# pierotofy/OpenSplat

Hardware: NVIDIA H100
Metric: fwd_bwd_mpixel_per_s (higher is better)
Workload: dtype f32

## Files before the change

### opensplat_b200/csrc/raster_bwd.cu

```cuda
#include "raster_common.cuh"

int gsb_blend_grid(const void *kernel, int num_tiles);

namespace {

__device__ __forceinline__ float rcp_approx(float x) {
    float y;
    asm("rcp.approx.ftz.f32 %0, %1;" : "=f"(y) : "f"(x));
    return y;
}

__device__ __forceinline__ void zero_row(float *grad_rows, int k) {
    float4 *row = reinterpret_cast<float4 *>(grad_rows + (size_t)k * GSB_GRAD_ROW_FLOATS);
    const float4 z = make_float4(0.f, 0.f, 0.f, 0.f);
    row[0] = z; row[1] = z; row[2] = z;
}

constexpr int BWD_MIN_BLOCKS = 6;
constexpr int BWD_DEPTH_MIN_BLOCKS = 5;
constexpr int BWD_ABS_MIN_BLOCKS = 5;
constexpr int BWD_DEPTH_ABS_MIN_BLOCKS = 4;
template <bool SAT, bool DEPTH, bool ABS>
__global__ void __launch_bounds__(RK_THREADS, ABS ? (DEPTH ? BWD_DEPTH_ABS_MIN_BLOCKS : BWD_ABS_MIN_BLOCKS)
                                                  : (DEPTH ? BWD_DEPTH_MIN_BLOCKS : BWD_MIN_BLOCKS))
rasterize_backward_kernel(int img_h, int img_w, int tiles_x, int num_tiles,
                          const int2 *__restrict__ tile_bins, const GsbRecord *__restrict__ records,
                          const float *__restrict__ background, const float *__restrict__ final_Ts,
                          const int *__restrict__ final_idx, const float *__restrict__ v_output,
                          const float *__restrict__ v_output_alpha, float *__restrict__ grad_rows,
                          unsigned *__restrict__ tile_counter, const int *__restrict__ tile_order,
                          const float *__restrict__ record_depths, const float *__restrict__ v_output_depth) {
    __shared__ WarpRing rings[RK_WARPS];
    const int warp = threadIdx.x >> 5, lane = threadIdx.x & 31;
    WarpRing &ring = rings[warp];
    if (lane == 0) {
#pragma unroll
        for (int s = 0; s < RK_STAGES; ++s) mbar_init(&ring.full[s], 1);
        mbar_fence_init();
    }
    __syncwarp();
    const float bg0 = __ldg(background), bg1 = __ldg(background + 1), bg2 = __ldg(background + 2);
    unsigned gchunk = 0;

    while (true) {
        int tile = 0;
        if (lane == 0) tile = (int)atomicAdd(tile_counter, 1u);
        tile = __shfl_sync(0xffffffffu, tile, 0);
        if (tile >= num_tiles) break;
        if (tile_order) tile = __ldg(tile_order + tile);
        const int2 range = tile_bins[tile];
        if (range.y <= range.x) continue;

        const int tx = tile % tiles_x, ty = tile / tiles_x;
        const int X = tx * GSB_TILE + (lane & 15);
        const int Y0 = ty * GSB_TILE + (lane >> 4);
        const float px = (float)X;
        const float tile_x0 = (float)(tx * GSB_TILE), tile_y0 = (float)(ty * GSB_TILE);

        float T[RK_PIX], Bq[RK_PIX];
        const float py0 = (float)Y0;
        float vor[RK_PIX], vog[RK_PIX], vob[RK_PIX];
        float vD[RK_PIX];
        int binf[RK_PIX];
        int my_max = -1;
#pragma unroll
        for (int j = 0; j < RK_PIX; ++j) {
            const int Y = Y0 + 2 * j;
            if (X < img_w && Y < img_h) {
                const size_t p = (size_t)Y * img_w + X;
                const float Tf = final_Ts[p];
                T[j] = Tf;
                vor[j] = v_output[3 * p]; vog[j] = v_output[3 * p + 1]; vob[j] = v_output[3 * p + 2];
                binf[j] = final_idx[p];
                if (SAT) {
                    const int f = binf[j];
                    if (f & GSB_SAT_BIT0) vor[j] = 0.f;
                    if (f & (GSB_SAT_BIT0 << 1)) vog[j] = 0.f;
                    if (f & (GSB_SAT_BIT0 << 2)) vob[j] = 0.f;
                    binf[j] = f & ~GSB_SAT_MASK;
                }
                if (DEPTH) vD[j] = v_output_depth ? v_output_depth[p] : 0.f;
                const float voa = v_output_alpha ? v_output_alpha[p] : 0.f;
                Bq[j] = -(Tf * (voa - (bg0 * vor[j] + bg1 * vog[j] + bg2 * vob[j])));
            } else {
                T[j] = 1.f; vor[j] = vog[j] = vob[j] = 0.f; Bq[j] = 0.f;
                if (DEPTH) vD[j] = 0.f;
                binf[j] = -1;
            }
            my_max = max(my_max, binf[j]);
        }
        const int warp_max = __reduce_max_sync(0xffffffffu, my_max);
        const int hi = min(range.y - 1, max(warp_max, range.x - 1));

        for (int idx = hi + 1 + lane; idx < range.y; idx += 32)
            zero_row(grad_rows, __float_as_int(__ldg(&records[idx].q0.w)));
        const int L = hi - range.x + 1;
        if (L <= 0) continue;
        const int nchunks = (L + RK_CHUNK - 1) / RK_CHUNK;

        const unsigned g0 = gchunk;
        auto stage_of = [&](int c) { return (g0 + (unsigned)c) % RK_STAGES; };
        auto parity_of = [&](int c) { return ((g0 + (unsigned)c) / RK_STAGES) & 1u; };
        auto chunk_lo = [&](int c) { return max(range.x, hi + 1 - (c + 1) * RK_CHUNK); };
        auto chunk_cnt = [&](int c) { return (hi + 1 - c * RK_CHUNK) - chunk_lo(c); };
        auto issue = [&](int c) {
            if (lane == 0) {
                const unsigned s = stage_of(c);
                const uint32_t bytes = (uint32_t)chunk_cnt(c) * (uint32_t)sizeof(GsbRecord);
                mbar_arrive_expect_tx(&ring.full[s], bytes);
                tma_load_1d(&ring.rec[s][0], records + chunk_lo(c), bytes, &ring.full[s]);
            }
        };
        const int pro = min(RK_STAGES, nchunks);
        for (int c = 0; c < pro; ++c) issue(c);
        int issued = pro;

        for (int c = 0; c < nchunks; ++c) {
            const unsigned s = stage_of(c);
            float zl = 0.f;
            if (DEPTH && lane < chunk_cnt(c)) zl = __ldg(record_depths + chunk_lo(c) + lane);
            mbar_wait(&ring.full[s], parity_of(c));
            const int lo = chunk_lo(c), cnt = chunk_cnt(c);
            unsigned my_mask = 0;
            if (lane < cnt) {
                my_mask = record_slot_mask(ring.rec[s][lane], tile_x0, tile_y0);
                if (my_mask == 0u) zero_row(grad_rows, __float_as_int(ring.rec[s][lane].q0.w));
            }
            unsigned live = __ballot_sync(0xffffffffu, my_mask != 0u);
            while (live) {
                const int t = 31 - __clz(live);
                live &= ~(1u << t);
                const unsigned rm = __shfl_sync(0xffffffffu, my_mask, t);
                float z = 0.f;
                if (DEPTH) z = __shfl_sync(0xffffffffu, zl, t);
                const int idx = lo + t;
                const float4 q0 = ring.rec[s][t].q0;
                const float4 q1 = ring.rec[s][t].q1;
                const float4 q2 = ring.rec[s][t].q2;
                const float smax = fmaxf(0.f, fmaf(q0.z, GSB_LN2, GSB_SMAX_BIAS));
                const float dx = q0.x - px;
                const float adx2 = q1.x * dx * dx;
                const float bdx = q1.y * dx;
                const float dy0 = q0.y - py0;
                float s0 = 0.f, s1 = 0.f, s2 = 0.f;
                float a_r = 0.f, a_g = 0.f, a_b = 0.f;
                float a_z = 0.f;
                float g_x = 0.f, g_y = 0.f;
                float adx = 0.f, c2 = 0.f;
                if (ABS) { adx = (2.f * q1.x) * dx; c2 = 2.f * q1.z; }
                bool any = false;
                const int jlo = __ffs(rm) - 1, jhi = 31 - __clz(rm);
#define GSB_BWD_SLOT(j)                                                                                   \
    {                                                                                                     \
        const float dy = dy0 - (float)(2 * j);                                                                      \
        const float sigma = fmaf(dy, fmaf(q1.z, dy, bdx), adx2);                                          \
        if (__float_as_uint(sigma) <= __float_as_uint(smax)) {                    \
            const float au = ex2_approx(fmaf(sigma, -GSB_LOG2E, q0.z));           \
            const float alpha = fminf(0.99f, au);                                                         \
            if (idx <= binf[j] && alpha >= (1.f / 255.f)) {                                               \
                any = true;                                                                               \
                const float ra = rcp_approx(1.f - alpha);                                                 \
                T[j] *= ra;                                                                               \
                const float fac = alpha * T[j];                                                           \
                a_r = fmaf(fac, vor[j], a_r);                                                             \
                a_g = fmaf(fac, vog[j], a_g);                                                             \
                a_b = fmaf(fac, vob[j], a_b);                                                             \
                if (DEPTH) a_z = fmaf(fac, vD[j], a_z);                                                   \
                float d = fmaf(q2.z, vob[j], fmaf(q2.y, vog[j], q2.x * vor[j]));         \
                if (DEPTH) d = fmaf(z, vD[j], d);                                        \
                const float v_alpha = fmaf(d, T[j], -(ra * Bq[j]));                                       \
                Bq[j] = fmaf(d, fac, Bq[j]);                                                              \
                 \
                const float w = au * v_alpha;                                                             \
                const float wdy = w * dy;                                                                 \
                s0 += w;                                                                                  \
                s1 += wdy;                                                                                \
                s2 = fmaf(wdy, dy, s2);                                                                   \
                if (ABS) {                                                                                \
                    g_x = fmaf(fabsf(w), fabsf(fmaf(q1.y, dy, adx)), g_x);                                \
                    g_y = fmaf(fabsf(w), fabsf(fmaf(c2, dy, bdx)), g_y);                                  \
                }                                                                                         \
            }                                                                                             \
        }                                                                                                 \
        if (jhi == j) break;                                                                              \
    }
                switch (jlo) {
                    case 0: GSB_BWD_SLOT(0)
                    case 1: GSB_BWD_SLOT(1)
                    case 2: GSB_BWD_SLOT(2)
                    case 3: GSB_BWD_SLOT(3)
                    case 4: GSB_BWD_SLOT(4)
                    case 5: GSB_BWD_SLOT(5)
                    case 6: GSB_BWD_SLOT(6)
                    default: GSB_BWD_SLOT(7)
                }
#undef GSB_BWD_SLOT
                const int k = __float_as_int(q0.w);
                float *row = grad_rows + (size_t)k * GSB_GRAD_ROW_FLOATS;
                if (!__any_sync(0xffffffffu, any)) {
                    if (lane < (ABS ? 12 : DEPTH ? 10 : 9)) row[lane] = 0.f;
                    continue;
                }
                const float sx = dx * s0;
                float v0 = s0, v1 = sx, v2 = s1, v3 = dx * sx, v4 = dx * s1, v5 = s2, v6 = a_r, v7 = a_g;
                float v8 = a_b;
                {
                    const bool up = lane & 16;
                    const float t0 = up ? v0 : v4, t1 = up ? v1 : v5, t2 = up ? v2 : v6, t3 = up ? v3 : v7;
                    const float k0 = up ? v4 : v0, k1 = up ? v5 : v1, k2 = up ? v6 : v2, k3 = up ? v7 : v3;
                    v0 = k0 + __shfl_xor_sync(0xffffffffu, t0, 16);
                    v1 = k1 + __shfl_xor_sync(0xffffffffu, t1, 16);
                    v2 = k2 + __shfl_xor_sync(0xffffffffu, t2, 16);
                    v3 = k3 + __shfl_xor_sync(0xffffffffu, t3, 16);
                }
                {
                    const bool up = lane & 8;
                    const float t0 = up ? v0 : v2, t1 = up ? v1 : v3;
                    const float k0 = up ? v2 : v0, k1 = up ? v3 : v1;
                    v0 = k0 + __shfl_xor_sync(0xffffffffu, t0, 8);
                    v1 = k1 + __shfl_xor_sync(0xffffffffu, t1, 8);
                }
                {
                    const bool up = lane & 4;
                    const float t0 = up ? v0 : v1;
                    const float k0 = up ? v1 : v0;
                    v0 = k0 + __shfl_xor_sync(0xffffffffu, t0, 4);
                }
                v0 += __shfl_xor_sync(0xffffffffu, v0, 2);
                v0 += __shfl_xor_sync(0xffffffffu, v0, 1);
                if (ABS) {
                    const bool up = lane & 16;
                    const float t8 = up ? v8 : a_z, k8 = up ? a_z : v8;
                    const float tg = up ? g_x : g_y, kg = up ? g_y : g_x;
                    v8 = k8 + __shfl_xor_sync(0xffffffffu, t8, 16);
                    const float e = kg + __shfl_xor_sync(0xffffffffu, tg, 16);
                    const bool up8 = lane & 8;
                    const float t = up8 ? v8 : e, kk = up8 ? e : v8;
                    v8 = kk + __shfl_xor_sync(0xffffffffu, t, 8);
#pragma unroll
                    for (int o = 4; o > 0; o >>= 1) v8 += __shfl_xor_sync(0xffffffffu, v8, o);
                    const bool wx = (lane & 7) == 1 && (DEPTH || lane != 17);
                    if (((lane & 3) == 0) || wx) row[wx ? 8 + ((lane >> 3) & 1) * 2 + (lane >> 4) : (lane >> 2)] =
                        wx ? v8 : v0;
                } else if (DEPTH) {
                    const bool up = lane & 16;
                    const float t8 = up ? v8 : a_z, k8 = up ? a_z : v8;
                    v8 = k8 + __shfl_xor_sync(0xffffffffu, t8, 16);
#pragma unroll
                    for (int o = 8; o > 0; o >>= 1) v8 += __shfl_xor_sync(0xffffffffu, v8, o);
                    const bool w8 = (lane == 1), w9 = (lane == 17);
                    if (((lane & 3) == 0) || w8 || w9) row[w8 ? 8 : w9 ? 9 : (lane >> 2)] = (w8 || w9) ? v8 : v0;
                } else {
#pragma unroll
                    for (int o = 16; o > 0; o >>= 1) v8 += __shfl_xor_sync(0xffffffffu, v8, o);
                    const bool w8 = (lane == 1);
                    if (((lane & 3) == 0) || w8) row[w8 ? 8 : (lane >> 2)] = w8 ? v8 : v0;
                }
            }
            __syncwarp();
            if (issued < nchunks) { issue(issued); ++issued; }
        }
        gchunk = g0 + (unsigned)issued;
        __syncwarp();
    }
}

template <bool DEPTH, bool ABS>
__global__ void __launch_bounds__(256)
reduce_grad_rows_kernel(int n, const int *__restrict__ cum_tiles_hit, const float *__restrict__ grad_rows,
                        const float *__restrict__ conics, const float *__restrict__ opacities,
                        float2 *__restrict__ v_xy, float *__restrict__ v_conic,
                        float *__restrict__ v_colors, float *__restrict__ v_opacity, float *__restrict__ v_depths,
                        float2 *__restrict__ v_xy_abs) {
    const int g = blockIdx.x * blockDim.x + threadIdx.x;
    if (g >= n) return;
    const int k0 = g ? cum_tiles_hit[g - 1] : 0, k1 = cum_tiles_hit[g];
    float a[9] = {0.f, 0.f, 0.f, 0.f, 0.f, 0.f, 0.f, 0.f, 0.f};
    float az = 0.f;
    float ax = 0.f, ay = 0.f;
    for (int k = k0; k < k1; ++k) {
        const float4 *row = reinterpret_cast<const float4 *>(grad_rows + (size_t)k * GSB_GRAD_ROW_FLOATS);
        const float4 r0 = row[0], r1 = row[1];
        a[0] += r0.x; a[1] += r0.y; a[2] += r0.z; a[3] += r0.w;
        a[4] += r1.x; a[5] += r1.y; a[6] += r1.z; a[7] += r1.w;
        if (ABS) {
            const float4 r2 = row[2];
            a[8] += r2.x;
            if (DEPTH) az += r2.y;
            ax += r2.z; ay += r2.w;
        } else {
            a[8] += reinterpret_cast<const float *>(row)[8];
            if (DEPTH) az += reinterpret_cast<const float *>(row)[9];
        }
    }
    const float S0 = a[0], Sx = a[1], Sy = a[2], Sxx = a[3], Sxy = a[4], Syy = a[5];
    const float ca = conics[3 * g], cb = conics[3 * g + 1], cc = conics[3 * g + 2];
    const float op = opacities[g];
    v_xy[g] = make_float2(-(ca * Sx + cb * Sy), -(cb * Sx + cc * Sy));
    v_conic[3 * g] = -0.5f * Sxx; v_conic[3 * g + 1] = -0.5f * Sxy; v_conic[3 * g + 2] = -0.5f * Syy;
    v_colors[3 * g] = a[6]; v_colors[3 * g + 1] = a[7]; v_colors[3 * g + 2] = a[8];
    v_opacity[g] = (op > 0.f) ? S0 / op : 0.f;
    if (DEPTH) v_depths[g] = az;
    if (ABS) v_xy_abs[g] = make_float2(ax, ay);
}

}

extern "C" size_t gsb_raster_grad_rows_bytes(int m) {
    return gsb_align_up((size_t)(m > 0 ? m : 0) * GSB_GRAD_ROW_FLOATS * 4 + 256, 256);
}

static int backward(int img_h, int img_w, int tiles_x, int tiles_y, int n, int m, const int32_t *tile_bins,
                    const int32_t *tile_order, const float *conics, const float *opacities, void *records,
                    const int32_t *cum_tiles_hit, const float *background, const float *final_Ts,
                    const int32_t *final_idx, const float *v_output, const float *v_output_alpha, void *grad_rows,
                    float *v_xy, float *v_conic, float *v_colors, float *v_opacity, unsigned flags, bool depth,
                    const float *record_depths, const float *v_output_depth, float *v_depths, float *v_xy_abs,
                    gsb_stream_t stream) {
    GSB_CHECK_ARG(img_h > 0 && img_w > 0 && n >= 0 && m >= 0);
    GSB_CHECK_ARG((flags & ~(unsigned)GSB_RASTER_CLAMP_MAX_ONE) == 0);
    const bool sat = (flags & GSB_RASTER_CLAMP_MAX_ONE) != 0;
    GSB_CHECK_ARG(tiles_x == gsb_div_up(img_w, GSB_TILE) && tiles_y == gsb_div_up(img_h, GSB_TILE));
    if (n == 0) return 0;
    GSB_CHECK_ARG(tile_bins && conics && opacities && cum_tiles_hit && background && final_Ts && final_idx &&
                  v_output && v_xy && v_conic && v_colors && v_opacity);
    GSB_CHECK_ARG(!depth || (v_depths && (record_depths || m == 0)));
    GSB_CHECK_ARG(((uintptr_t)v_xy % 8) == 0 && ((uintptr_t)v_xy_abs % 8) == 0);
    const bool abs = v_xy_abs != nullptr;
    cudaStream_t s = (cudaStream_t)stream;
    if (m > 0) {
        GSB_CHECK_ARG(records && grad_rows && ((uintptr_t)records % 16) == 0 && ((uintptr_t)grad_rows % 16) == 0);
        unsigned *counters = reinterpret_cast<unsigned *>(
            reinterpret_cast<char *>(records) + gsb_raster_records_bytes(m) - 256);
        GSB_CUDA(cudaMemsetAsync(counters, 0, 256, s));
        const int num_tiles = tiles_x * tiles_y;
#define GSB_BWD_LAUNCH(S, D, A)                                                                                 \
    rasterize_backward_kernel<S, D, A><<<gsb_blend_grid((const void *)rasterize_backward_kernel<S, D, A>,       \
                                                        num_tiles), RK_THREADS, 0, s>>>(                        \
        img_h, img_w, tiles_x, num_tiles, reinterpret_cast<const int2 *>(tile_bins),                            \
        reinterpret_cast<const GsbRecord *>(records), background, final_Ts, final_idx, v_output, v_output_alpha, \
        reinterpret_cast<float *>(grad_rows), counters, tile_order, record_depths, v_output_depth)
        if (abs) {
            if (depth) {
                if (sat) GSB_BWD_LAUNCH(true, true, true); else GSB_BWD_LAUNCH(false, true, true);
            } else {
                if (sat) GSB_BWD_LAUNCH(true, false, true); else GSB_BWD_LAUNCH(false, false, true);
            }
        } else if (depth) {
            if (sat) GSB_BWD_LAUNCH(true, true, false); else GSB_BWD_LAUNCH(false, true, false);
        } else {
            if (sat) GSB_BWD_LAUNCH(true, false, false); else GSB_BWD_LAUNCH(false, false, false);
        }
#undef GSB_BWD_LAUNCH
    }
#define GSB_REDUCE_LAUNCH(D, A)                                                                                 \
    reduce_grad_rows_kernel<D, A><<<gsb_div_up(n, 256), 256, 0, s>>>(                                           \
        n, cum_tiles_hit, reinterpret_cast<const float *>(grad_rows), conics, opacities,                        \
        reinterpret_cast<float2 *>(v_xy), v_conic, v_colors, v_opacity, v_depths,                               \
        reinterpret_cast<float2 *>(v_xy_abs))
    if (abs) {
        if (depth) GSB_REDUCE_LAUNCH(true, true); else GSB_REDUCE_LAUNCH(false, true);
    } else if (depth) {
        GSB_REDUCE_LAUNCH(true, false);
    } else {
        GSB_REDUCE_LAUNCH(false, false);
    }
#undef GSB_REDUCE_LAUNCH
    GSB_LAUNCH_CHECK();
    return 0;
}

extern "C" int gsb_rasterize_backward(int img_h, int img_w, int tiles_x, int tiles_y, int n, int m,
                                      const int32_t *tile_bins, const int32_t *tile_order, const float *conics,
                                      const float *opacities, void *records, const int32_t *cum_tiles_hit,
                                      const float *background, const float *final_Ts, const int32_t *final_idx,
                                      const float *v_output, const float *v_output_alpha, void *grad_rows,
                                      float *v_xy, float *v_conic, float *v_colors, float *v_opacity, unsigned flags,
                                      gsb_stream_t stream) {
    return backward(img_h, img_w, tiles_x, tiles_y, n, m, tile_bins, tile_order, conics, opacities, records,
                    cum_tiles_hit, background, final_Ts, final_idx, v_output, v_output_alpha, grad_rows, v_xy, v_conic,
                    v_colors, v_opacity, flags, false, nullptr, nullptr, nullptr, nullptr, stream);
}

extern "C" int gsb_rasterize_backward_depth(int img_h, int img_w, int tiles_x, int tiles_y, int n, int m,
                                            const int32_t *tile_bins, const int32_t *tile_order, const float *conics,
                                            const float *opacities, void *records, const int32_t *cum_tiles_hit,
                                            const float *background, const float *final_Ts, const int32_t *final_idx,
                                            const float *v_output, const float *v_output_alpha, void *grad_rows,
                                            float *v_xy, float *v_conic, float *v_colors, float *v_opacity,
                                            unsigned flags, const float *record_depths, const float *v_output_depth,
                                            float *v_depths, gsb_stream_t stream) {
    return backward(img_h, img_w, tiles_x, tiles_y, n, m, tile_bins, tile_order, conics, opacities, records,
                    cum_tiles_hit, background, final_Ts, final_idx, v_output, v_output_alpha, grad_rows, v_xy, v_conic,
                    v_colors, v_opacity, flags, true, record_depths, v_output_depth, v_depths, nullptr, stream);
}

extern "C" int gsb_rasterize_backward_absgrad(int img_h, int img_w, int tiles_x, int tiles_y, int n, int m,
                                              const int32_t *tile_bins, const int32_t *tile_order,
                                              const float *conics, const float *opacities, void *records,
                                              const int32_t *cum_tiles_hit, const float *background,
                                              const float *final_Ts, const int32_t *final_idx, const float *v_output,
                                              const float *v_output_alpha, void *grad_rows, float *v_xy,
                                              float *v_conic, float *v_colors, float *v_opacity, unsigned flags,
                                              const float *record_depths, const float *v_output_depth,
                                              float *v_depths, float *v_xy_abs, gsb_stream_t stream) {
    GSB_CHECK_ARG(v_xy_abs != nullptr);
    GSB_CHECK_ARG(v_depths || (!record_depths && !v_output_depth));
    return backward(img_h, img_w, tiles_x, tiles_y, n, m, tile_bins, tile_order, conics, opacities, records,
                    cum_tiles_hit, background, final_Ts, final_idx, v_output, v_output_alpha, grad_rows, v_xy, v_conic,
                    v_colors, v_opacity, flags, v_depths != nullptr, record_depths, v_output_depth, v_depths, v_xy_abs,
                    stream);
}
```

### opensplat_b200/csrc/raster_common.cuh

```cuda
#pragma once
#include "gsb_common.cuh"

struct __align__(16) GsbRecord {
    float4 q0, q1, q2;
};
static_assert(sizeof(GsbRecord) == 48, "record must be 48 bytes");

constexpr int RK_WARPS = 4;
constexpr int RK_THREADS = RK_WARPS * 32;
constexpr int RK_PIX = 8;
constexpr int RK_CHUNK = 32;
constexpr int RK_STAGES = 4;

constexpr float GSB_LN2 = 0.6931471805599453f;
constexpr float GSB_LOG2E = 1.4426950408889634f;
constexpr float GSB_SMAX_BIAS = 5.541263545158426f + 1e-3f;

constexpr int GSB_GRAD_ROW_FLOATS = 12;

constexpr int GSB_SAT_BIT0 = 1 << 28;
constexpr int GSB_SAT_MASK = 7 << 28;

struct __align__(128) WarpRing {
    GsbRecord rec[RK_STAGES][RK_CHUNK];
    uint64_t full[RK_STAGES];
};

#ifdef __CUDACC__
__device__ __forceinline__ GsbRecord make_record(float2 xy, float a, float b, float c, float opac, float r,
                                                 float g, float bl, int k) {
    const float lo = (opac > 0.f) ? log2f(opac) : -INFINITY;
    const float smax = fmaxf(0.f, fmaf(lo, GSB_LN2, GSB_SMAX_BIAS));
    const float det = a * c - b * b;
    float hx = INFINITY, hy = INFINITY;
    if (det > 0.f && a > 0.f && c > 0.f) {
        const float s2 = 2.f * smax / det;
        hx = sqrtf(s2 * c) * 1.001f + 0.01f;
        hy = sqrtf(s2 * a) * 1.001f + 0.01f;
    }
    GsbRecord rec;
    rec.q0 = make_float4(xy.x, xy.y, lo, __int_as_float(k));
    rec.q1 = make_float4(0.5f * a, b, 0.5f * c, hx);
    rec.q2 = make_float4(r, g, bl, hy);
    return rec;
}

__device__ __forceinline__ unsigned extent_slot_mask(float cx, float cy, float hx, float hy, float tile_x0,
                                                     float tile_y0) {
    const float gx = cx - tile_x0, gy = cy - tile_y0;
    const float xlo = fmaxf(ceilf(gx - hx), 0.f), xhi = fminf(floorf(gx + hx), 15.f);
    const float ylo = fmaxf(ceilf(gy - hy), 0.f), yhi = fminf(floorf(gy + hy), 15.f);
    if (!(xlo <= xhi) || !(ylo <= yhi)) return 0u;
    const int jlo = (int)ylo >> 1, jhi = (int)yhi >> 1;
    return ((2u << jhi) - 1u) & ~((1u << jlo) - 1u);
}

__device__ __forceinline__ unsigned record_slot_mask(const GsbRecord &r, float tile_x0, float tile_y0) {
    return extent_slot_mask(r.q0.x, r.q0.y, r.q1.w, r.q2.w, tile_x0, tile_y0);
}
#endif
```

Before: 1093.

## Split backward warp into half-tiles processing two gaussians concurrently

Remaps each warp so the two 16-lane halves cover the left and right 8-column halves of the tile, and uses an x-extent bit in the slot mask to let each half walk its own list of live gaussians. Each half reduces its partial gradients with shuffles, stages them in a new shared-memory partials buffer, and a final per-record pass combines the left and right halves and writes grad rows as float4 stores. This replaces per-gaussian row zeroing and scattered scalar writes. It aims to cut wasted lanes on gaussians that only touch one half of the tile, at the cost of extra shared memory and a lower min-blocks launch bound.

```diff
diff --git a/opensplat_b200/csrc/raster_bwd.cu b/opensplat_b200/csrc/raster_bwd.cu
--- a/opensplat_b200/csrc/raster_bwd.cu
+++ b/opensplat_b200/csrc/raster_bwd.cu
@@ -16,9 +16,9 @@
     row[0] = z; row[1] = z; row[2] = z;
 }
 
-constexpr int BWD_MIN_BLOCKS = 6;
-constexpr int BWD_DEPTH_MIN_BLOCKS = 5;
-constexpr int BWD_ABS_MIN_BLOCKS = 5;
+constexpr int BWD_MIN_BLOCKS = 5;
+constexpr int BWD_DEPTH_MIN_BLOCKS = 4;
+constexpr int BWD_ABS_MIN_BLOCKS = 4;
 constexpr int BWD_DEPTH_ABS_MIN_BLOCKS = 4;
 template <bool SAT, bool DEPTH, bool ABS>
 __global__ void __launch_bounds__(RK_THREADS, ABS ? (DEPTH ? BWD_DEPTH_ABS_MIN_BLOCKS : BWD_ABS_MIN_BLOCKS)
@@ -30,9 +30,14 @@
                           const float *__restrict__ v_output_alpha, float *__restrict__ grad_rows,
                           unsigned *__restrict__ tile_counter, const int *__restrict__ tile_order,
                           const float *__restrict__ record_depths, const float *__restrict__ v_output_depth) {
+    constexpr int NV = ABS ? 12 : DEPTH ? 10 : 9;
+    constexpr int PS = NV | 1;
     __shared__ WarpRing rings[RK_WARPS];
+    __shared__ float partials[RK_WARPS][2][RK_CHUNK * PS];
     const int warp = threadIdx.x >> 5, lane = threadIdx.x & 31;
+    const int half = lane >> 4, hl = lane & 15;
     WarpRing &ring = rings[warp];
+    float *const my_part = partials[warp][half];
     if (lane == 0) {
 #pragma unroll
         for (int s = 0; s < RK_STAGES; ++s) mbar_init(&ring.full[s], 1);
@@ -52,8 +57,8 @@
         if (range.y <= range.x) continue;
 
         const int tx = tile % tiles_x, ty = tile / tiles_x;
-        const int X = tx * GSB_TILE + (lane & 15);
-        const int Y0 = ty * GSB_TILE + (lane >> 4);
+        const int X = tx * GSB_TILE + 8 * half + (lane & 7);
+        const int Y0 = ty * GSB_TILE + ((lane >> 3) & 1);
         const float px = (float)X;
         const float tile_x0 = (float)(tx * GSB_TILE), tile_y0 = (float)(ty * GSB_TILE);
 
@@ -122,15 +127,18 @@
             mbar_wait(&ring.full[s], parity_of(c));
             const int lo = chunk_lo(c), cnt = chunk_cnt(c);
             unsigned my_mask = 0;
-            if (lane < cnt) {
-                my_mask = record_slot_mask(ring.rec[s][lane], tile_x0, tile_y0);
-                if (my_mask == 0u) zero_row(grad_rows, __float_as_int(ring.rec[s][lane].q0.w));
-            }
-            unsigned live = __ballot_sync(0xffffffffu, my_mask != 0u);
-            while (live) {
-                const int t = 31 - __clz(live);
-                live &= ~(1u << t);
-                const unsigned rm = __shfl_sync(0xffffffffu, my_mask, t);
+            if (lane < cnt) my_mask = record_slot_half_mask(ring.rec[s][lane], tile_x0, tile_y0);
+            unsigned liveL = __ballot_sync(0xffffffffu, my_mask & 0x100u);
+            unsigned liveR = __ballot_sync(0xffffffffu, my_mask & 0x200u);
+            while (liveL | liveR) {
+                const int tL = 31 - __clz(liveL), tR = 31 - __clz(liveR);
+                if (liveL) liveL &= ~(1u << tL);
+                if (liveR) liveR &= ~(1u << tR);
+                const int tm = half ? tR : tL;
+                const int t = max(tm, 0);
+                const unsigned rs = __shfl_sync(0xffffffffu, my_mask, t);
+                const unsigned rm = tm >= 0 ? (rs & 0xffu) : 0u;
+                const unsigned rmU = __reduce_or_sync(0xffffffffu, rm);
                 float z = 0.f;
                 if (DEPTH) z = __shfl_sync(0xffffffffu, zl, t);
                 const int idx = lo + t;
@@ -149,12 +157,12 @@
                 float adx = 0.f, c2 = 0.f;
                 if (ABS) { adx = (2.f * q1.x) * dx; c2 = 2.f * q1.z; }
                 bool any = false;
-                const int jlo = __ffs(rm) - 1, jhi = 31 - __clz(rm);
+                const int jlo = __ffs(rmU) - 1, jhi = 31 - __clz(rmU);
 #define GSB_BWD_SLOT(j)                                                                                   \
     {                                                                                                     \
-        const float dy = dy0 - (float)(2 * j);                                                                      \
+        const float dy = dy0 - (float)(2 * j);                                  \
         const float sigma = fmaf(dy, fmaf(q1.z, dy, bdx), adx2);                                          \
-        if (__float_as_uint(sigma) <= __float_as_uint(smax)) {                    \
+        if ((rm & (1u << j)) && __float_as_uint(sigma) <= __float_as_uint(smax)) {  \
             const float au = ex2_approx(fmaf(sigma, -GSB_LOG2E, q0.z));           \
             const float alpha = fminf(0.99f, au);                                                         \
             if (idx <= binf[j] && alpha >= (1.f / 255.f)) {                                               \
@@ -195,67 +203,76 @@
                     default: GSB_BWD_SLOT(7)
                 }
 #undef GSB_BWD_SLOT
-                const int k = __float_as_int(q0.w);
-                float *row = grad_rows + (size_t)k * GSB_GRAD_ROW_FLOATS;
-                if (!__any_sync(0xffffffffu, any)) {
-                    if (lane < (ABS ? 12 : DEPTH ? 10 : 9)) row[lane] = 0.f;
-                    continue;
+                float out = 0.f, out_e = 0.f;
+                if (__any_sync(0xffffffffu, any)) {
+                    const float sx = dx * s0;
+                    float v0 = s0, v1 = sx, v2 = s1, v3 = dx * sx, v4 = dx * s1, v5 = s2, v6 = a_r, v7 = a_g;
+                    {
+                        const bool up = lane & 8;
+                        const float t0 = up ? v0 : v4, t1 = up ? v1 : v5, t2 = up ? v2 : v6, t3 = up ? v3 : v7;
+                        const float k0 = up ? v4 : v0, k1 = up ? v5 : v1, k2 = up ? v6 : v2, k3 = up ? v7 : v3;
+                        v0 = k0 + __shfl_xor_sync(0xffffffffu, t0, 8);
+                        v1 = k1 + __shfl_xor_sync(0xffffffffu, t1, 8);
+                        v2 = k2 + __shfl_xor_sync(0xffffffffu, t2, 8);
+                        v3 = k3 + __shfl_xor_sync(0xffffffffu, t3, 8);
+                    }
+                    {
+                        const bool up = lane & 4;
+                        const float t0 = up ? v0 : v2, t1 = up ? v1 : v3;
+                        const float k0 = up ? v2 : v0, k1 = up ? v3 : v1;
+                        v0 = k0 + __shfl_xor_sync(0xffffffffu, t0, 4);
+                        v1 = k1 + __shfl_xor_sync(0xffffffffu, t1, 4);
+                    }
+                    {
+                        const bool up = lane & 2;
+                        const float t0 = up ? v0 : v1;
+                        const float k0 = up ? v1 : v0;
+                        v0 = k0 + __shfl_xor_sync(0xffffffffu, t0, 2);
+                    }
+                    out = v0 + __shfl_xor_sync(0xffffffffu, v0, 1);
+                    float e = a_b;
+                    int o = 8;
+                    if (ABS) {
+                        const bool up = lane & 8;
+                        const float t0 = up ? a_b : g_x, t1 = up ? a_z : g_y;
+                        const float k0 = up ? g_x : a_b, k1 = up ? g_y : a_z;
+                        const float x0 = k0 + __shfl_xor_sync(0xffffffffu, t0, 8);
+                        const float x1 = k1 + __shfl_xor_sync(0xffffffffu, t1, 8);
+                        const bool up4 = lane & 4;
+                        e = (up4 ? x1 : x0) + __shfl_xor_sync(0xffffffffu, up4 ? x0 : x1, 4);
+                        o = 2;
+                    } else if (DEPTH) {
+                        const bool up = lane & 8;
+                        e = (up ? a_z : a_b) + __shfl_xor_sync(0xffffffffu, up ? a_b : a_z, 8);
+                        o = 4;
+                    }
+#pragma unroll
+                    for (; o > 0; o >>= 1) e += __shfl_xor_sync(0xffffffffu, e, o);
+                    out_e = e;
                 }
-                const float sx = dx * s0;
-                float v0 = s0, v1 = sx, v2 = s1, v3 = dx * sx, v4 = dx * s1, v5 = s2, v6 = a_r, v7 = a_g;
-                float v8 = a_b;
-                {
-                    const bool up = lane & 16;
-                    const float t0 = up ? v0 : v4, t1 = up ? v1 : v5, t2 = up ? v2 : v6, t3 = up ? v3 : v7;
-                    const float k0 = up ? v4 : v0, k1 = up ? v5 : v1, k2 = up ? v6 : v2, k3 = up ? v7 : v3;
-                    v0 = k0 + __shfl_xor_sync(0xffffffffu, t0, 16);
-                    v1 = k1 + __shfl_xor_sync(0xffffffffu, t1, 16);
-                    v2 = k2 + __shfl_xor_sync(0xffffffffu, t2, 16);
-                    v3 = k3 + __shfl_xor_sync(0xffffffffu, t3, 16);
+                constexpr int esh = ABS ? 2 : DEPTH ? 3 : 4;
+                const bool st_e = (hl & ((1 << esh) - 1)) == 1;
+                if (rm && (!(hl & 1) || st_e)) my_part[t * PS + (st_e ? 8 + (hl >> esh) : hl >> 1)] = st_e ? out_e : out;
+            }
+            __syncwarp();
+            if (lane < cnt) {
+                const float *pl = partials[warp][0] + lane * PS, *pr = partials[warp][1] + lane * PS;
+                const bool inL = my_mask & 0x100u, inR = my_mask & 0x200u;
+                float r[GSB_GRAD_ROW_FLOATS];
+#pragma unroll
+                for (int v = 0; v < GSB_GRAD_ROW_FLOATS; ++v) {
+                    float a = 0.f;
+                    if (v < NV) {
+                        if (inL) a = pl[v];
+                        if (inR) a = inL ? a + pr[v] : pr[v];
+                    }
+                    r[v] = a;
                 }
-                {
-                    const bool up = lane & 8;
-                    const float t0 = up ? v0 : v2, t1 = up ? v1 : v3;
-                    const float k0 = up ? v2 : v0, k1 = up ? v3 : v1;
-                    v0 = k0 + __shfl_xor_sync(0xffffffffu, t0, 8);
-                    v1 = k1 + __shfl_xor_sync(0xffffffffu, t1, 8);
-                }
-                {
-                    const bool up = lane & 4;
-                    const float t0 = up ? v0 : v1;
-                    const float k0 = up ? v1 : v0;
-                    v0 = k0 + __shfl_xor_sync(0xffffffffu, t0, 4);
-                }
-                v0 += __shfl_xor_sync(0xffffffffu, v0, 2);
-                v0 += __shfl_xor_sync(0xffffffffu, v0, 1);
-                if (ABS) {
-                    const bool up = lane & 16;
-                    const float t8 = up ? v8 : a_z, k8 = up ? a_z : v8;
-                    const float tg = up ? g_x : g_y, kg = up ? g_y : g_x;
-                    v8 = k8 + __shfl_xor_sync(0xffffffffu, t8, 16);
-                    const float e = kg + __shfl_xor_sync(0xffffffffu, tg, 16);
-                    const bool up8 = lane & 8;
-                    const float t = up8 ? v8 : e, kk = up8 ? e : v8;
-                    v8 = kk + __shfl_xor_sync(0xffffffffu, t, 8);
-#pragma unroll
-                    for (int o = 4; o > 0; o >>= 1) v8 += __shfl_xor_sync(0xffffffffu, v8, o);
-                    const bool wx = (lane & 7) == 1 && (DEPTH || lane != 17);
-                    if (((lane & 3) == 0) || wx) row[wx ? 8 + ((lane >> 3) & 1) * 2 + (lane >> 4) : (lane >> 2)] =
-                        wx ? v8 : v0;
-                } else if (DEPTH) {
-                    const bool up = lane & 16;
-                    const float t8 = up ? v8 : a_z, k8 = up ? a_z : v8;
-                    v8 = k8 + __shfl_xor_sync(0xffffffffu, t8, 16);
-#pragma unroll
-                    for (int o = 8; o > 0; o >>= 1) v8 += __shfl_xor_sync(0xffffffffu, v8, o);
-                    const bool w8 = (lane == 1), w9 = (lane == 17);
-                    if (((lane & 3) == 0) || w8 || w9) row[w8 ? 8 : w9 ? 9 : (lane >> 2)] = (w8 || w9) ? v8 : v0;
-                } else {
-#pragma unroll
-                    for (int o = 16; o > 0; o >>= 1) v8 += __shfl_xor_sync(0xffffffffu, v8, o);
-                    const bool w8 = (lane == 1);
-                    if (((lane & 3) == 0) || w8) row[w8 ? 8 : (lane >> 2)] = w8 ? v8 : v0;
-                }
+                const int k = __float_as_int(ring.rec[s][lane].q0.w);
+                float4 *row = reinterpret_cast<float4 *>(grad_rows + (size_t)k * GSB_GRAD_ROW_FLOATS);
+                row[0] = make_float4(r[0], r[1], r[2], r[3]);
+                row[1] = make_float4(r[4], r[5], r[6], r[7]);
+                row[2] = make_float4(r[8], r[9], r[10], r[11]);
             }
             __syncwarp();
             if (issued < nchunks) { issue(issued); ++issued; }
diff --git a/opensplat_b200/csrc/raster_common.cuh b/opensplat_b200/csrc/raster_common.cuh
--- a/opensplat_b200/csrc/raster_common.cuh
+++ b/opensplat_b200/csrc/raster_common.cuh
@@ -45,17 +45,25 @@
     return rec;
 }
 
-__device__ __forceinline__ unsigned extent_slot_mask(float cx, float cy, float hx, float hy, float tile_x0,
-                                                     float tile_y0) {
+__device__ __forceinline__ unsigned extent_slot_half_mask(float cx, float cy, float hx, float hy, float tile_x0,
+                                                          float tile_y0) {
     const float gx = cx - tile_x0, gy = cy - tile_y0;
     const float xlo = fmaxf(ceilf(gx - hx), 0.f), xhi = fminf(floorf(gx + hx), 15.f);
     const float ylo = fmaxf(ceilf(gy - hy), 0.f), yhi = fminf(floorf(gy + hy), 15.f);
     if (!(xlo <= xhi) || !(ylo <= yhi)) return 0u;
     const int jlo = (int)ylo >> 1, jhi = (int)yhi >> 1;
-    return ((2u << jhi) - 1u) & ~((1u << jlo) - 1u);
+    return (((2u << jhi) - 1u) & ~((1u << jlo) - 1u)) | (xlo <= 7.f ? 0x100u : 0u) | (xhi >= 8.f ? 0x200u : 0u);
+}
+
+__device__ __forceinline__ unsigned extent_slot_mask(float cx, float cy, float hx, float hy, float tile_x0,
+                                                     float tile_y0) {
+    return extent_slot_half_mask(cx, cy, hx, hy, tile_x0, tile_y0) & 0xffu;
 }
 
 __device__ __forceinline__ unsigned record_slot_mask(const GsbRecord &r, float tile_x0, float tile_y0) {
     return extent_slot_mask(r.q0.x, r.q0.y, r.q1.w, r.q2.w, tile_x0, tile_y0);
 }
+__device__ __forceinline__ unsigned record_slot_half_mask(const GsbRecord &r, float tile_x0, float tile_y0) {
+    return extent_slot_half_mask(r.q0.x, r.q0.y, r.q1.w, r.q2.w, tile_x0, tile_y0);
+}
 #endif
```

Measured after the change: 1070 (median of 6 runs). 2.2% lower.
